# acproject/wsi-segmentation-pipeline

Measured on AMD Instinct MI355X. Metric: patches/sec (256×256×3) whole-slide inference, 1/2/4/8 MI355X + CPU ref, higher is better.
Workload: dtype fp16 + MX-fp6 cross terms (fp32 accumulate); 1 GPU; cfg3: ONE 40000x40000 synthetic slide, tile 256 stride 256 -> 24648 tiles sharded over 1 rank(s) (each holds only its own slide regions: 4.80 GB on rank 0), ResNet-18 trunk + Classifier, fused read+normalise+conv HIP path, 1 all-gather, float64 stitch + softmax; tiles_total=24648, batch=6200, mode=mx, parallelism=tile-shard x1 + 1 all-gather, batches_in_flight=2

## Files before the change

wsi_segmentation_pipeline_amd/csrc/conv.hip:

```cpp
#include "conv_dev.h"
#include "internal.h"

template <int MT, int WM, int WN, int PLANES, bool POST = false>
__global__ __launch_bounds__(WM* WN * 64) void conv_gather_kernel(ConvArgs a) {
    extern __shared__ __attribute__((aligned(16))) char smem[];
    constexpr int BM = WM * MT * 32;
    constexpr int NTHREADS = WM * WN * 64;
    constexpr int PPT = BM * 8 / NTHREADS;
    constexpr int PIX_STEP = NTHREADS / 8;
    const int tid = threadIdx.x, lane = tid & 63, wave = tid >> 6;
    const int wm = wave / WN, wn = wave % WN;
    const int l31 = lane & 31, h = lane >> 5;
    const int nblocks = a.go.C / (WN * 32);
    const int nb = blockIdx.x % nblocks;
    const int mtile = blockIdx.x / nblocks;
    const int q0 = a.go.G + mtile * BM;
    const int ntile = nb * WN + wn;
    const int NC = a.gi.C / PFmt<PLANES>::CPL;
    const int KS = a.ksize, NT = KS * KS, pad = KS / 2;
    const size_t in_pixstride = (size_t)a.gi.C * PFmt<PLANES>::BPC;
    const bf16x8* wbase = (const bf16x8*)a.wpk + (size_t)ntile * NC * NT * 4 * 64 + lane;

    int inq[PPT];
    const int sp = tid & 7;
// ... 22 lines not shown
    for (int c = 0; c < NC; ++c) {
        for (int t = 0; t < NT; ++t) {
            const int toff = (t / KS) * a.gi.P + (t % KS);
            __syncthreads();
#pragma unroll
            for (int k = 0; k < PPT; ++k) {
                const int m = (tid >> 3) + k * PIX_STEP;
                const int s = sp ^ ((m >> 1) & 7);
                const int src = inq[k] < 0 ? 0 : inq[k] + toff;
                *(uint4*)(smem + (size_t)(m * 8 + sp) * 16) =
                    *(const uint4*)((const char*)a.in + (size_t)src * in_pixstride + c * 128 + s * 16);
            }
            bf16x8 wf[4];
#pragma unroll
            for (int f = 0; f < 4; ++f) wf[f] = wbase[((size_t)(c * NT + t) * 4 + f) * 64];
            __syncthreads();
            mfma_line<MT, PLANES>(acc, wf, smem, xbase);
        }
    }
    conv_epilogue<MT, PLANES, POST>(a, acc, q0 + wm * MT * 32, ntile, lane);
}

#ifdef WSI_STUDY
__device__ unsigned long long g_wide_stamps[8];
#define WSTAMP(...) __VA_ARGS__
extern "C" int wsi_study_wide_stamps(unsigned long long* out8, int reset) {
    if (out8 && hipMemcpyFromSymbol(out8, HIP_SYMBOL(g_wide_stamps), sizeof(g_wide_stamps)) != hipSuccess) return WSI_EFAULT;
    if (reset) {
        unsigned long long z[8] = {0};
        if (hipMemcpyToSymbol(HIP_SYMBOL(g_wide_stamps), z, sizeof(z)) != hipSuccess) return WSI_EFAULT;
    }
    return WSI_OK;
}
static __device__ __forceinline__ void wide_stamps_report(int lane, unsigned long long st_begin, unsigned long long st_setup, unsigned long long st_pro,
                                                          unsigned long long st_line, unsigned long long st_tap, unsigned long long st_loop_end) {
    asm volatile("s_waitcnt vmcnt(0)" ::: "memory");
    if (lane == 0 && (blockIdx.x & 63) == 0) {
        const unsigned long long st_end = __builtin_readcyclecounter();
        atomicAdd(&g_wide_stamps[0], 1ull);
        atomicAdd(&g_wide_stamps[1], st_end - st_begin);
        atomicAdd(&g_wide_stamps[2], st_setup - st_begin);
        atomicAdd(&g_wide_stamps[3], st_pro);
        atomicAdd(&g_wide_stamps[4], st_line);
        atomicAdd(&g_wide_stamps[5], st_tap);
        atomicAdd(&g_wide_stamps[6], st_end - st_loop_end);
    }
}
#else
#define WSTAMP(...)
#endif


template <int MT, int WM, int WN, int PLANES, int MINW, bool DENSE, int ABL = 0, bool PAIR = false>
__global__ __launch_bounds__(WM* WN * 64, MINW) void conv3x3s1_slab3_kernel(ConvArgs a) {
    extern __shared__ __attribute__((aligned(16))) char smem[];
    constexpr int BM = WM * MT * 32;
    constexpr int NTHREADS = WM * WN * 64;
    constexpr int RESID_NBUF = MT < 2 ? MT : 2;
    constexpr bool SCHED = MINW < 3;
    const int tid = threadIdx.x, lane = tid & 63;
    if (CONV_STUDY(a, CONV_ABL_DISPATCH_ONLY)) return;
    WSTAMP(const unsigned long long st_begin = __builtin_readcyclecounter(); unsigned long long st_pro = 0, st_line = 0, st_tap = 0, st_a = 0;)
    const int wave = __builtin_amdgcn_readfirstlane(tid >> 6);
    const int wm = wave / WN, wn = wave % WN;
    const int l31 = lane & 31, h = lane >> 5;
    const int nblocks = a.go.C / (WN * 32);
    int nb, mtile;
    if (!conv_tile_of_block(a.flags, nblocks, DENSE ? (a.gi.N * a.gi.H * a.gi.W + BM - 1) / BM : (a.gi.NS + BM - 1) / BM, nb, mtile)) return;
// ... 101 lines not shown
                const int k = t * MT + mt;
                if constexpr (!(ABL & 32)) {
                    if (mt + 1 < MT) xload_m(xf[(k + 1) & 1], xoff[mt + 1] + toff, mt + 1);
                    else if (t < 8) xload_m(xf[(k + 1) & 1], xoff[0] + toff_next, 0);
                }
                if constexpr (SCHED) __builtin_amdgcn_sched_barrier(0);
                const bf16x8(&w)[4] = wbuf[t % 3];
                const bf16x8(&x)[4] = xf[k & 1];
                if constexpr (ABL & 8) {
#pragma unroll
                    for (int f = 0; f < 4; ++f) acc[0][mt][f] += (float)w[f][0] * (float)x[f][0];
                } else if constexpr (PLANES == 3) {
                    acc[0][mt] = mfma_mx6(acc[0][mt], w, x);
                } else if constexpr (PLANES == 2) {
                    mfma_step<2>(acc[0][mt], w, x);
                } else {
#pragma unroll
                    for (int f = 0; f < 4; ++f) acc[0][mt] = mfma_bf16(w[f], x[f], acc[0][mt]);
                }
                if constexpr (SCHED) __builtin_amdgcn_sched_barrier(0);
            }
        }
    }
    WSTAMP(const unsigned long long st_loop_end = __builtin_readcyclecounter();)
    if constexpr (PLANES == 3) {
        if (a.resid) __syncthreads();
        conv_tail_mx<1, MT, RESID_NBUF>(a, acc, qs, valid, ntile, lane, smem + wave * (RESID_NBUF * 4096), slab0);
    } else {
        char* scratch = nullptr;
        if (PLANES == 2 && a.resid && !(a.flags & CONV_RESID_DIRECT)) {
            __syncthreads();
            scratch = smem + wave * 8192;
        }
        conv_epilogue_q<MT, PLANES>(a, acc[0], qs, valid, ntile, lane, scratch);
    }
    WSTAMP(wide_stamps_report(lane, st_begin, st_setup, st_pro, st_line, st_tap, st_loop_end);)
}

long long dense_max_slab_pixels(const ConvArgs& a, int BM) {
    const long long R = (long long)a.gi.N * a.gi.H * a.gi.W;
    const int mtiles = (int)((R + BM - 1) / BM);
    const int HW = a.gi.H * a.gi.W;
    auto pos = [&](long long i) { const long long n = i / HW, rem = i - n * HW; return (long long)a.gi.G + n * a.gi.S + (rem / a.gi.W) * a.gi.P + rem % a.gi.W; };
    auto span = [&](int m) { const long long i0 = (long long)m * BM, i1 = (i0 + BM < R ? i0 + BM : R) - 1; return pos(i1) + a.gi.P + 1 - (pos(i0) - a.gi.P - 1) + 1; };
    long long maxpix = span(mtiles - 1);
    int g = BM, r = HW;
    while (r) { const int t = g % r; g = r; r = t; }
    const int period = HW / g + 1;
    const int scan = mtiles < period ? mtiles : period;
    for (int m = 0; m < scan; ++m) { const long long px = span(m); if (px > maxpix) maxpix = px; }
    return maxpix;
}

size_t conv_slab_lds(long long maxpix, int nthreads, int waves) {
    const size_t lds = (size_t)((maxpix * 8 + nthreads - 1) / nthreads * nthreads) * 16;
    return lds < (size_t)waves * 8192 ? (size_t)waves * 8192 : lds;
}
int conv_grid(int mtiles, int nblocks, int flags) {
    return (flags & CONV_XCD_ORDER) ? (mtiles + 7) / 8 * 8 * nblocks : (flags & CONV_XCD_RANGES) ? (mtiles * nblocks + 7) / 8 * 8 : mtiles * nblocks;
// ... 10 lines not shown
        mtiles = (int)((R + BM - 1) / BM);
        maxpix = (int)dense_max_slab_pixels(a, BM);
    } else {
        mtiles = (a.gi.NS + BM - 1) / BM;
        maxpix = BM + 2 * a.gi.P + 2;
    }
    const size_t lds = conv_slab_lds(maxpix, NTHREADS, WM * WN);
    if (lds > 160 * 1024) return WSI_EINVAL;
    if (PAIR && (!DENSE || MT % 2 || a.gi.W % 64 || ((long long)a.gi.N * a.gi.H * a.gi.W) % BM)) return WSI_EINVAL;
    if (a.in_up) {
        constexpr int CPL = PFmt<PLANES>::CPL;
        if (a.up_c <= 0 || a.up_c % CPL || a.up_c > a.gi.C || (a.up_c < a.gi.C && !a.in) || a.gup.H * 2 != a.gi.H || a.gup.W * 2 != a.gi.W ||
            a.gup.N != a.gi.N || (a.flags & (CONV_IN96 | CONV_RESID96)) || a.in2 ||
            (size_t)pf_alloc_pixels(a.gup.N, a.gup.H, a.gup.W) * a.up_c * PFmt<PLANES>::BPC > (size_t)0x7fffffff)
            return WSI_EINVAL;
    }
    return conv_launch(conv3x3s1_slab3_kernel<MT, WM, WN, PLANES, MINW, DENSE, ABL, PAIR>, conv_grid(mtiles, nblocks, a.flags), NTHREADS, lds, st, a);
}


template <int MINW, int NCT = 0, bool IN96 = true>
__global__ __launch_bounds__(256, MINW) void conv3x3s1_rows_kernel(ConvArgs a) {
    extern __shared__ __attribute__((aligned(16))) char smem[];
    constexpr int MT = 4, WN = 2, BM = 256, NTHREADS = 256, RESID_NBUF = 2;
    const int tid = threadIdx.x, lane = tid & 63;
    WSTAMP(const unsigned long long st_begin = __builtin_readcyclecounter(); unsigned long long st_pro = 0, st_line = 0, st_tap = 0, st_a = 0;)
    const int wave = __builtin_amdgcn_readfirstlane(tid >> 6);
    const int wm = wave / WN, wn = wave % WN;
    const int l31 = lane & 31, h = lane >> 5;
    const int nblocks = a.go.C / (WN * 32);
    int nb, mtile;
    if (!conv_tile_of_block(a.flags & CONV_XCD_RANGES, nblocks, (a.gi.N * a.gi.H * a.gi.W) / BM, nb, mtile)) return;
    const int P = a.gi.P;
    const int ntile = nb * WN + wn;
    const int NC = NCT ? NCT : a.gi.C / 32;
    constexpr bool in96 = IN96;
    const size_t in_pixstride = in96 ? (size_t)96 : (size_t)a.gi.C * 4;
    const int in_line = in96 ? 0 : 128;
    const int p0 = pf_pos_of_index(a.gi, mtile * BM);
    const int slab0 = p0 - P - 1;
    const int npieces = (5 * P + 66) * 8;
    const int xoff0 = wm * 32 + l31;
    const size_t slab_byte0 = (size_t)slab0 * in_pixstride, in_bytes = (size_t)pf_alloc_pixels(a.gi.N, a.gi.H, a.gi.W) * in_pixstride;
    const __amdgpu_buffer_rsrc_t xrs = slab_rsrc(a.in, slab_byte0, in_bytes);
    bool xact;
    const int xvoff = slab_lane_voff96(wave * 64 + lane, (int)in_pixstride, in96, xact);
    const __amdgpu_buffer_rsrc_t wrs = __builtin_amdgcn_make_buffer_rsrc(
// ... 46 lines not shown
        if (c == 0) acc_init_bias<MT>(acc[0], a.bias, ntile, lane);
        xload(xf[0], xoff0);
#pragma unroll
        for (int dx = 0; dx < 3; ++dx) {
#pragma unroll
            for (int j = 0; j < 6; ++j) {
                const int k = dx * 6 + j;
                if (j < 5) xload(xf[(k + 1) & 1], xoff0 + (j + 1) * Pc + dx);
                else if (dx < 2) xload(xf[(k + 1) & 1], xoff0 + dx + 1);
                __builtin_amdgcn_sched_barrier(0);
#pragma unroll
                for (int mt = 0; mt < MT; ++mt) {
                    const int dy = j - mt;
                    if (dy >= 0 && dy < 3) acc[0][mt] = mfma_mx6(acc[0][mt], wbuf[dy], xf[k & 1]);
                }
                __builtin_amdgcn_sched_barrier(0);
                if (j >= 3 && (dx < 2 || (XLINE && c + 1 < NC))) {
                    wload(wbuf[j - 3], dx < 2 ? sline + ((j - 3) * 3 + dx + 1) * 4096 : sline + (9 + (j - 3) * 3) * 4096);
                    __builtin_amdgcn_sched_barrier(0);
                }
            }
        }
    }
    WSTAMP(const unsigned long long st_loop_end = __builtin_readcyclecounter();)
    int qs[MT];
    bool valid[MT];
#pragma unroll
    for (int mt = 0; mt < MT; ++mt) {
        qs[mt] = p0 + mt * P + wm * 32 + l31;
        valid[mt] = true;
    }
    if (a.resid) __syncthreads();
    conv_tail_mx<1, MT, RESID_NBUF>(a, acc, qs, valid, ntile, lane, smem + wave * (RESID_NBUF * 4096), slab0);
    WSTAMP(wide_stamps_report(lane, st_begin, st_setup, st_pro, st_line, st_tap, st_loop_end);)
}

template <int MINW>
static int launch_rows(const ConvArgs& a, hipStream_t st) {
    const bool nc2 = a.gi.C == 64;
    constexpr int BM = 256, NTHREADS = 256;
    if (a.go.C % 64 || a.gi.C % 32 || a.gi.W != 64 || a.gi.H % 4 || a.in2) return WSI_EINVAL;
    const int nblocks = a.go.C / 64;
    const long long R = (long long)a.gi.N * a.gi.H * a.gi.W;
    const int mtiles = (int)(R / BM);
    const size_t lds = conv_slab_lds(5 * a.gi.P + 66, NTHREADS, 4);
    const bool i96 = a.flags & CONV_IN96;
    auto k = nc2 ? (i96 ? conv3x3s1_rows_kernel<MINW, 2, true> : conv3x3s1_rows_kernel<MINW, 2, false>)
                 : (i96 ? conv3x3s1_rows_kernel<MINW, 0, true> : conv3x3s1_rows_kernel<MINW, 0, false>);
    return conv_launch(k, conv_grid(mtiles, nblocks, a.flags & CONV_XCD_RANGES), NTHREADS, lds, st, a);
}


constexpr int L1P_SLAB_PIX = 392;
constexpr int L1P_SLAB = L1P_SLAB_PIX * 128;
constexpr int L1P_STAGE = 16 * 3072;
constexpr int L1P_LDS = 2 * L1P_SLAB + L1P_STAGE;
template <int NCT>
// ... 329 lines not shown
#pragma unroll
            for (int mt = 0; mt < MT; ++mt) {
                const int k = t * MT + mt;
                if constexpr (!(ABL & 32)) {
                    if (mt + 1 < MT) xload(xf[(k + 1) & 1], xoff[mt + 1] + toff, t % 3);
                    else if (t < 8) xload(xf[(k + 1) & 1], xoff[0] + toff_next, (t + 1) % 3);
                }
                __builtin_amdgcn_sched_barrier(0);
                const bf16x8(&x)[4] = xf[k & 1];
#pragma unroll
                for (int nt = 0; nt < NT; ++nt) {
                    mfma_step<PLANES>(acc[nt][mt], wf[nt], x);
                }
            }
            if (t < 8) {
                WSTAMP(st_a = __builtin_readcyclecounter();)
                asm volatile("s_waitcnt vmcnt(0)" ::: "memory");
                __syncthreads();
                WSTAMP(st_tap += __builtin_readcyclecounter() - st_a;)
            }
            kpar ^= 1;
        }
    }
    WSTAMP(const unsigned long long st_loop_end = __builtin_readcyclecounter();)
    int qs[MT];
#pragma unroll
    for (int mt = 0; mt < MT; ++mt) {
        if constexpr (D8) {
            const int i = mtile * BM + wm * MT * 32 + mt * 32 + lpix;
            qs[mt] = pf_pos_of_index(a.gi, valid[mt] ? i : min(mtile * BM + BM, Rtot) - 1);
        } else {
            qs[mt] = xoff[mt] + slab0 + (P + 1);
        }
    }
    if constexpr (PLANES == 3) {
        if (a.in2) {
            const int NC2 = a.in2_c / 32;
            const size_t ps2 = (size_t)a.in2_c * 4;
            const __amdgpu_buffer_rsrc_t xrs2 = slab_rsrc(a.in2, (size_t)slab0 * ps2, (size_t)pf_alloc_pixels(a.gi.N, a.gi.H, a.gi.W) * ps2);
            const int xvoff2 = lane_voff((int)ps2);
            const char* wsrc2 = (const char*)a.wpk2 + (size_t)(nb * NTILES) * NC2 * 4096 + (size_t)(tid & 255) * 16;
#pragma unroll
            for (int nt = 0; nt < NT; ++nt) {
                f32x16 b2[1];
                acc_init_bias<1>(b2, a.bias2, nb * NTILES + wn * NT + nt, lane);
#pragma unroll
                for (int mt = 0; mt < MT; ++mt)
// ... 3 lines not shown
            for (int c = 0; c < NC2; ++c) {
                __syncthreads();
                slab_dma_rounds<NTHREADS, false>(xrs2, xl, wave, npieces, xvoff2, c * 128, RPIX * (int)ps2);
#pragma unroll
                for (int p0 = 0; p0 < NTILES * 256; p0 += NTHREADS) {
                    const int pw = p0 + wave * 64;
                    dma16(wsrc2 + (size_t)((pw >> 8) * NC2 + c) * 4096, wl + pw * 16);
                }
                asm volatile("s_waitcnt vmcnt(0)" ::: "memory");
                __syncthreads();
                bf16x8 wf2[NT][4];
#pragma unroll
                for (int nt = 0; nt < NT; ++nt) wread(wf2[nt], wl, nt);
#pragma unroll
                for (int mt = 0; mt < MT; ++mt) {
                    bf16x8 x2[4];
                    xload(x2, xoff[mt] + (D8 ? 8 : P) + 1);
#pragma unroll
                    for (int nt = 0; nt < NT; ++nt) mfma_step<PLANES>(acc[nt][mt], wf2[nt], x2);
                }
            }
        }
        if (a.resid) __syncthreads();
        conv_tail_mx<NT, MT, RESID_NBUF>(a, acc, qs, valid, nb * NTILES + wn * NT, lane, smem + wave * (RESID_NBUF * 4096), slab0);
    } else {
        char* scratch = nullptr;
        if (PLANES == 2 && a.resid && !(a.flags & CONV_RESID_DIRECT)) {
            __syncthreads();
            scratch = xl + wave * 8192;
        }
#pragma unroll
        for (int nt = 0; nt < NT; ++nt) conv_epilogue_q<MT, PLANES>(a, acc[nt], qs, valid, nb * NTILES + wn * NT + nt, lane, scratch);
    }
    WSTAMP(wide_stamps_report(lane, st_begin, st_setup, st_pro, st_line, st_tap, st_loop_end);)
}


template <int PLANES, int MINW, int ABL = 0, int WM = 2, int WN = 2, int NT = 2, bool D8 = false>
static int launch_wide(const ConvArgs& a, hipStream_t st) {
    constexpr int BM = WM * 128, NTHREADS = WM * WN * 64, BN = WN * NT * 32;
    if (a.go.C % BN) return WSI_EINVAL;
    if constexpr (!D8 && ABL == 0 && WM == 2 && WN == 2 && NT == 2) {
        if (g_routes.wide_d8 && a.gi.W == 8 && a.gi.H == 8) return launch_wide<PLANES, MINW, 0, 2, 2, 2, true>(a, st);
    }
    const int nblocks = a.go.C / BN;
    const long long R = (long long)a.gi.N * a.gi.H * a.gi.W;
    const int mtiles = (int)((R + BM - 1) / BM);
    const size_t xbytes = D8 ? (size_t)(304 + 16) * 128
                             : conv_slab_lds(dense_max_slab_pixels(a, BM), NTHREADS, WM * WN);
    size_t lds = 2 * (BN / 32) * 4096 + xbytes;
    if (PLANES == 3 && lds < (size_t)WM * WN * 4 * 4096) lds = (size_t)WM * WN * 4 * 4096;
    if (lds > 160 * 1024) return WSI_EINVAL;
    return conv_launch(conv3x3s1_wide_kernel<PLANES, MINW, ABL, WM, WN, NT, D8>, conv_grid(mtiles, nblocks, a.flags & CONV_XCD_RANGES), NTHREADS, lds, st, a);
}


template <int MT, int WM, int WN, int PLANES, int MINW, bool FUSE, int PMAX = 34, int ABL = 0>
// ... 471 lines not shown
```

wsi_segmentation_pipeline_amd/csrc/conv_dev.h:

```cpp
#pragma once
#include "common.h"

static __device__ __forceinline__ void dma16(const void* gsrc, char* lds_wave_base) {
    __builtin_amdgcn_global_load_lds((const __attribute__((address_space(1))) void*)gsrc,
                                     (__attribute__((address_space(3))) void*)lds_wave_base, 16, 0, 0);
}

static __device__ __forceinline__ void dma16_buf(__amdgpu_buffer_rsrc_t rs, char* lds_wave_base, int voff, int soff) {
    __builtin_amdgcn_raw_ptr_buffer_load_lds(rs, (__attribute__((address_space(3))) void*)lds_wave_base, 16, voff, soff, 0, 0);
}

static __device__ __forceinline__ unsigned lds_addr_of(const char* p) {
    return (unsigned)(size_t)(const __attribute__((address_space(3))) char*)p;
}
static __device__ __forceinline__ void dma16_asm(const void* gsrc, unsigned lds) {
    unsigned keep;
    asm volatile("s_mov_b32 %0, m0\n\ts_mov_b32 m0, %1\n\ts_nop 0\n\tglobal_load_lds_dwordx4 %2, off\n\ts_mov_b32 m0, %0"
                 : "=&s"(keep) : "s"(lds), "v"(gsrc) : "memory");
}
static __device__ __forceinline__ void dma16_buf_asm(__amdgpu_buffer_rsrc_t rs, unsigned lds, int voff, int soff) {
    unsigned keep;
    asm volatile("s_mov_b32 %0, m0\n\ts_mov_b32 m0, %1\n\ts_nop 0\n\tbuffer_load_dwordx4 %2, %3, %4 offen lds\n\ts_mov_b32 m0, %0"
                 : "=&s"(keep) : "s"(lds), "v"(voff), "s"(rs), "s"(soff) : "memory");
}

static __device__ __forceinline__ void resid_tile_dma(const void* resid, int q_own, size_t pixstride, size_t line_off, int lane, char* dst) {
#pragma unroll
    for (int j = 0; j < 4; ++j) {
        const int pp = 8 * j + (lane >> 3);
        const int q = __shfl(q_own, pp);
        const int sl = (lane & 7) ^ ((pp >> 1) & 7);
        dma16((const char*)resid + (size_t)q * pixstride + line_off + sl * 16, dst + j * 1024);
    }
}

static __device__ __forceinline__ void resid_tile_dma_buf(__amdgpu_buffer_rsrc_t rs, int q_rel, int pixstride, int line_off, int lane, char* dst) {
#pragma unroll
    for (int j = 0; j < 4; ++j) {
        const int pp = 8 * j + (lane >> 3);
        const int q = __shfl(q_rel, pp);
        const int sl = (lane & 7) ^ ((pp >> 1) & 7);
        dma16_buf(rs, dst + j * 1024, q * pixstride + sl * 16, line_off);
    }
}

static __device__ __forceinline__ bool mx96_stored(int s) { return s != 5 && s != 7; }
static __device__ __forceinline__ int mx96_piece(int s) { return s == 6 ? 5 : s; }

static __device__ __forceinline__ void mx96_rebuild_hi6(char* slab, int npix, int tid, int nthreads) {
    for (int Pl = tid; Pl < npix; Pl += nthreads) {
        const int key = (Pl >> 1) & 7;
        char* line = slab + Pl * 128;
        unsigned D[16];
#pragma unroll
        for (int s4 = 0; s4 < 4; ++s4) {
            const u32x4 d = *(const u32x4*)(line + ((s4 ^ key) << 4));
            D[4 * s4] = d[0]; D[4 * s4 + 1] = d[1]; D[4 * s4 + 2] = d[2]; D[4 * s4 + 3] = d[3];
        }
        const int sh = (int)(*(const unsigned*)(line + ((6 ^ key) << 4) + 12) & 255u);
        u32x16 e;
#pragma unroll
        for (int k = 0; k < 16; ++k)
            e[k] = __builtin_amdgcn_perm(D[8 + (k >> 1)], D[k >> 1], (k & 1) ? 0x07060302u : 0x05040100u);
        u32x6 q;
        const float scale = sh ? mx_scale_value(sh) : 1.f;
        asm volatile("v_cvt_scalef32_pk32_fp6_f16 %0, %1, %2" : "=&v"(q) : "v"(e), "v"(scale));
        *(u32x4*)(line + ((5 ^ key) << 4)) = u32x4{q[0], q[1], q[2], q[3]};
        *(u32x4*)(line + ((7 ^ key) << 4)) = u32x4{q[4], q[5], (unsigned)sh, 0u};
    }
}

static __device__ __forceinline__ void resid_tile_dma_buf96(__amdgpu_buffer_rsrc_t rs, int q_rel, int pixstride, int line_off, int lane, char* dst) {
#pragma unroll
    for (int j = 0; j < 4; ++j) {
        const int pp = 8 * j + (lane >> 3);
        const int q = __shfl(q_rel, pp);
        const int sl = (lane & 7) ^ ((pp >> 1) & 7);
        if (mx96_stored(sl)) dma16_buf(rs, dst + j * 1024, q * pixstride + mx96_piece(sl) * 16, line_off);
    }
}

template <int MT, int PLANES, bool POST = false>
static __device__ __forceinline__ void conv_epilogue_q(const ConvArgs& a, f32x16 (&acc)[MT], const int (&qs)[MT],
                                                       const bool (&valid)[MT], int ntile, int lane, char* scratch = nullptr) {
    typedef typename PairElem<PLANES>::T E;
    typedef __attribute__((ext_vector_type(4))) E Ex4;
    const int h = lane >> 5, l31 = lane & 31;
    const size_t pixstride = (size_t)a.go.C * PFmt<PLANES>::BPC;
    const size_t chan_off = (size_t)ntile * (32 * PFmt<PLANES>::BPC) + (size_t)(4 * h) * 2;
    size_t poff[MT], ooff[MT];
#pragma unroll
    for (int mt = 0; mt < MT; ++mt) {
        poff[mt] = (size_t)(valid[mt] ? qs[mt] : a.go.G) * pixstride + chan_off;
        ooff[mt] = a.out_split_pixels ? pf_out_offset(a.go, a.out_split_pixels, valid[mt] ? qs[mt] : a.go.G, pixstride) + chan_off : poff[mt];
    }

    const bool via_lds = PLANES == 2 && a.resid && scratch;
    Ex4 rh[MT][4], rl[MT][4];
    if (via_lds) {
        resid_tile_dma(a.resid, valid[0] ? qs[0] : a.go.G, pixstride, (size_t)ntile * 128, lane, scratch);
    } else if (a.resid) {
// ... 100 lines not shown
    d = __builtin_amdgcn_mfma_f32_32x32x16_f16(__builtin_bit_cast(f16x8, w[1]), __builtin_bit_cast(f16x8, x[1]), d, 0, 0, 0);
    const i32x4 wq = __builtin_bit_cast(i32x4, w[2]), wr = __builtin_bit_cast(i32x4, w[3]);
    const i32x4 xq = __builtin_bit_cast(i32x4, x[2]), xr = __builtin_bit_cast(i32x4, x[3]);
    const i32x8 wa = {wq[0], wq[1], wq[2], wq[3], wr[0], wr[1], wr[2], wr[3]}, xa = {xq[0], xq[1], xq[2], xq[3], xr[0], xr[1], xr[2], xr[3]};
    return __builtin_amdgcn_mfma_scale_f32_32x32x64_f8f6f4(wa, xa, d, 2, 2, 0, wr[2], 0, xr[2]);
}

template <int MT>
static __device__ __forceinline__ void acc_init_bias(f32x16 (&acc)[MT], const float* bias, int ntile, int lane) {
    const int h = lane >> 5;
    float b[16];
#pragma unroll
    for (int g = 0; g < 4; ++g) {
        const f32x4 v = *(const f32x4*)(bias + ntile * 32 + 8 * g + 4 * h);
#pragma unroll
        for (int i = 0; i < 4; ++i) b[4 * g + i] = v[i];
    }
#pragma unroll
    for (int mt = 0; mt < MT; ++mt)
#pragma unroll
        for (int r = 0; r < 16; ++r) acc[mt][r] = b[r];
}

template <int MT, int MTN = MT>
static __device__ __forceinline__ void conv_epilogue_mx(const ConvArgs& a, f32x16 (&acc)[MT], const int (&qs)[MT],
                                                        const bool (&valid)[MT], int ntile, int lane, int mt0 = 0) {
    const int h = lane >> 5;
    const bool o96 = a.flags & CONV_OUT96;
    const size_t pixstride = o96 ? (size_t)96 : (size_t)a.go.C * 4;
    const float lo_clamp = a.relu ? 0.f : -65504.f;
#pragma unroll
    for (int mt = mt0; mt < mt0 + MTN; ++mt) {
        const size_t loff = (size_t)(valid[mt] ? qs[mt] : a.go.G) * pixstride + (o96 ? (size_t)ntile * (size_t)a.plane96 : (size_t)ntile * 128);
        f32x16 v = acc[mt];
        f32x16 hi, lo;
        f16x8 hv[2];
        float mv = 0.f, ml = 0.f;
#pragma unroll
        for (int r = 0; r < 16; r += 2) {
            const float v0 = __builtin_amdgcn_fmed3f(v[r], lo_clamp, 65504.f);
            const float v1 = __builtin_amdgcn_fmed3f(v[r + 1], lo_clamp, 65504.f);
            const f16x2 hh = __builtin_convertvector(f32x2{v0, v1}, f16x2);
            hv[r >> 3][r & 7] = hh[0];
            hv[r >> 3][(r & 7) + 1] = hh[1];
            hi[r] = (float)hh[0];
            hi[r + 1] = (float)hh[1];
            lo[r] = v0 - hi[r];
            lo[r + 1] = v1 - hi[r + 1];
            mv = fmaxf(mv, fmaxf(fabsf(hi[r]), fabsf(hi[r + 1])));
            ml = fmaxf(ml, fmaxf(fabsf(lo[r]), fabsf(lo[r + 1])));
        }
        pair_max2(mv, ml);
        const int sh = mx6_scale_byte(mv), sl = mx6_scale_byte(ml);
        const int sb = h ? sh : sl;
        swap32_halves(lo, hi);
        const u32x6 q = mx6_pack32(lo, hi, sb ? mx_scale_value(sb) : 1.f);
        if (valid[mt] && !CONV_STUDY(a, CONV_ABL_NO_STORE)) {
            char* ol = (char*)a.out + (a.out_split_pixels ? pf_out_offset(a.go, a.out_split_pixels, qs[mt], pixstride) + (size_t)ntile * 128 : loff);
            *(f16x8*)(ol + 32 * h) = hv[0];
            *(f16x8*)(ol + 32 * h + 16) = hv[1];
            if (!o96) {
                *(u32x4*)(ol + MX6_PLANE_LO(0) + 16 * h) = u32x4{q[0], q[1], q[2], q[3]};
                *(u32x4*)(ol + MX6_PLANE_HI(0) + 16 * h) = u32x4{q[4], q[5], (unsigned)sb, 0u};
            } else if (h == 0) {
                *(u32x4*)(ol + 64) = u32x4{q[0], q[1], q[2], q[3]};
                *(u32x4*)(ol + 80) = u32x4{q[4], q[5], (unsigned)sl, (unsigned)sh};
            }
        }
    }
}

template <int NT, int MT, int NBUF>
static __device__ __forceinline__ void conv_tail_mx(const ConvArgs& a, f32x16 (&acc)[NT][MT], const int (&qs)[MT], const bool (&valid)[MT],
                                                    int ntile0, int lane, char* scratch, int slab0) {
    constexpr int T = NT * MT;
    static_assert(MT % NBUF == 0 || NBUF % MT == 0, "a batch is part of one channel tile or whole channel tiles");
    static_assert(NBUF <= T && T % NBUF == 0, "whole batches");
    if (!a.resid) {
#pragma unroll
        for (int nt = 0; nt < NT; ++nt) conv_epilogue_mx<MT>(a, acc[nt], qs, valid, ntile0 + nt, lane);
        return;
    }
    const int h = lane >> 5, l31 = lane & 31;
    const bool r96 = a.flags & CONV_RESID96;
    const int pixstride = r96 ? 96 : a.go.C * 4;
    const size_t rbase = (size_t)slab0 * pixstride, rbytes = (size_t)pf_alloc_pixels(a.go.N, a.go.H, a.go.W) * pixstride;
    const __amdgpu_buffer_rsrc_t rrs = __builtin_amdgcn_make_buffer_rsrc((void*)((const char*)a.resid + rbase), 0,
                                                                          (int)min(rbytes - rbase, (size_t)0x7fffffff), 0x00020000);
    bf16x8 iw[4];
    {
        const int p = mx_line_pos(l31), f0 = mx6_field_of_pos(p);
        f16x8 k0, k1;
#pragma unroll
        for (int j = 0; j < 8; ++j) {
            k0[j] = (p == 8 * h + j) ? (_Float16)1.0f : (_Float16)0.0f;
            k1[j] = (p == 16 + 8 * h + j) ? (_Float16)1.0f : (_Float16)0.0f;
        }
        unsigned q[6];
#pragma unroll
        for (int d = 0; d < 6; ++d) {
            const int bit = 6 * f0 + 3 - 32 * d;
            q[d] = (h == 0 && bit >= 0 && bit < 32) ? (1u << (bit & 31)) : 0u;
        }
        iw[0] = __builtin_bit_cast(bf16x8, k0);
        iw[1] = __builtin_bit_cast(bf16x8, k1);
        iw[2] = __builtin_bit_cast(bf16x8, u32x4{q[0], q[1], q[2], q[3]});
        iw[3] = __builtin_bit_cast(bf16x8, u32x4{q[4], q[5], 127u, 0u});
    }
    auto rdma = [&](int k) {
        const int nt = k / MT, mt = k % MT;
        int qr = qs[mt] - slab0;
        asm volatile("" : "+v"(qr));
        if (r96) {
            const __amdgpu_buffer_rsrc_t prs = __builtin_amdgcn_make_buffer_rsrc(
                (void*)((const char*)a.resid + (size_t)(ntile0 + nt) * (size_t)a.plane96 + rbase), 0, (int)min(rbytes - rbase, (size_t)0x7fffffff), 0x00020000);
            resid_tile_dma_buf96(prs, qr, pixstride, 0, lane, scratch + (k % NBUF) * 4096);
        }
        else resid_tile_dma_buf(rrs, qr, pixstride, (ntile0 + nt) * 128, lane, scratch + (k % NBUF) * 4096);
    };
    const int xb = l31 * 128 + ((h ^ ((l31 >> 1) & 7)) << 4);
#pragma unroll
    for (int k = 0; k < NBUF; ++k) rdma(k);
#pragma unroll
    for (int b0 = 0; b0 < T; b0 += NBUF) {
        asm volatile("s_waitcnt vmcnt(0)" ::: "memory");
#pragma unroll
        for (int k = b0; k < b0 + NBUF; ++k) {
            const char* t = scratch + (k % NBUF) * 4096;
            bf16x8 x[4];
#pragma unroll
            for (int f = 0; f < 4; ++f) x[f] = *(const bf16x8*)(t + (xb ^ (f << 5)));
            if (r96 && h) {
                x[2] = __builtin_bit_cast(bf16x8, u32x4{0u, 0u, 0u, 0u});
                x[3] = x[2];
            }
            acc[k / MT][k % MT] = mfma_mx6(acc[k / MT][k % MT], iw, x);
        }
        if (b0 + NBUF < T) {
            asm volatile("s_waitcnt lgkmcnt(0)" ::: "memory");
#pragma unroll
            for (int k = b0 + NBUF; k < b0 + 2 * NBUF; ++k) rdma(k);
        }
        if constexpr (NBUF >= MT) {
#pragma unroll
            for (int nt = b0 / MT; nt < (b0 + NBUF) / MT; ++nt) conv_epilogue_mx<MT>(a, acc[nt], qs, valid, ntile0 + nt, lane);
        } else {
            conv_epilogue_mx<MT, NBUF>(a, acc[b0 / MT], qs, valid, ntile0 + b0 / MT, lane, b0 % MT);
        }
    }
}

template <int MT, int PLANES, bool POST = false>
static __device__ __forceinline__ void conv_epilogue(const ConvArgs& a, f32x16 (&acc)[MT], int q_base, int ntile,
                                                     int lane) {
    int qs[MT];
    bool valid[MT];
#pragma unroll
    for (int mt = 0; mt < MT; ++mt) {
        qs[mt] = q_base + mt * 32 + (lane & 31);
        valid[mt] = pf_is_pixel(a.go, qs[mt]);
    }
    conv_epilogue_q<MT, PLANES, POST>(a, acc, qs, valid, ntile, lane);
}

template <int MT, int PLANES>
static __device__ __forceinline__ void conv_epilogue_any(const ConvArgs& a, f32x16 (&acc)[MT], int q_base, int ntile, int lane) {
    if constexpr (PLANES == 3) {
        int qs[MT];
        bool valid[MT];
#pragma unroll
// ... 144 lines not shown
```

wsi_segmentation_pipeline_amd/csrc/conv_pp.hip:

```cpp
#include "conv_dev.h"
#include "internal.h"

#define PP_BARRIER() do { asm volatile("s_waitcnt lgkmcnt(0)\n\ts_barrier" ::: "memory"); __builtin_amdgcn_sched_barrier(0); } while (0)
#define PP_BARRIER_VM() do { asm volatile("s_waitcnt vmcnt(0) lgkmcnt(0)\n\ts_barrier" ::: "memory"); __builtin_amdgcn_sched_barrier(0); } while (0)

#ifdef WSI_STUDY
#define PP_STAMP(x) do { if constexpr (STAMP) { unsigned long long t_; asm volatile("s_memtime %0\n\ts_waitcnt lgkmcnt(0)" : "=s"(t_) :: "memory"); x; } } while (0)
#else
#define PP_STAMP(x) do { } while (0)
#endif

template <int PLANES, int WM, int WN, int MT, bool STAMP = false, int DMODE = 0, bool PRIO = false>
__global__ __launch_bounds__(512, 2) void conv3x3s1_pp_kernel(ConvArgs a, int xbytes) {
    extern __shared__ __attribute__((aligned(16))) char smem[];
    constexpr int NT = 2, BM = WM * MT * 32, NTILES = WN * NT, WB = NTILES * 4096;
    constexpr int NF = 4;
    constexpr int RESID_NBUF = 4;
    static_assert(WM * WN == 8, "eight waves: two groups of four, one wave of each group per SIMD");
    char* const wl = smem;
    char* const xl = smem + 2 * WB;
    const int tid = threadIdx.x, lane = tid & 63;
    const int wave = __builtin_amdgcn_readfirstlane(tid >> 6);
    const int grp = wave >> 2;
    const int wm = wave / WN, wn = wave % WN;
// ... 114 lines not shown
            for (int mt = 0; mt < MT; ++mt)
#pragma unroll
                for (int nt = 0; nt < NT; ++nt) mfma_step<PLANES>(acc[nt][mt], wf[nt], xf[mt]);
#pragma unroll
            for (int mt = 0; mt < MT; ++mt) asm volatile("" : "+v"(acc[0][mt]), "+v"(acc[1][mt]));
            if constexpr (PRIO) __builtin_amdgcn_s_setprio(0);
            PP_STAMP(tsum[2] += t_ - tprev; tprev = t_);
            if (grp == 0 && DMODE != 1) asm volatile("s_waitcnt vmcnt(0)" ::: "memory");
            PP_BARRIER();
            PP_STAMP(tsum[3] += t_ - tprev; tprev = t_);
        }
    }
#ifdef WSI_STUDY
    if constexpr (STAMP) {
        if ((blockIdx.x == 0 || blockIdx.x == 300) && lane == 0 && a.out2) {
            unsigned long long* o = (unsigned long long*)a.out2 + ((blockIdx.x ? 1 : 0) * 8 + wave) * 6;
            for (int k = 0; k < 6; ++k) o[k] = tsum[k];
        }
    }
#endif
    if (grp == 0) PP_BARRIER();
    if constexpr (PLANES == 3) {
        constexpr int NBUF = RESID_NBUF % MT ? MT : (RESID_NBUF < NT * MT ? RESID_NBUF : NT * MT);
        conv_tail_mx<NT, MT, NBUF>(a, acc, qs, valid, nb * NTILES + wn * NT, lane, smem + wave * (RESID_NBUF * 4096), slab0);
    } else {
        char* scratch = nullptr;
        if (PLANES == 2 && a.resid && !(a.flags & CONV_RESID_DIRECT)) scratch = xl + wave * 8192;
#pragma unroll
        for (int nt = 0; nt < NT; ++nt) conv_epilogue_q<MT, PLANES>(a, acc[nt], qs, valid, nb * NTILES + wn * NT + nt, lane, scratch);
    }
}

template <int PLANES, int WM, int WN, int MT, bool STAMP = false, int DMODE = 0, bool PRIO = false>
static int launch_pp(const ConvArgs& a, hipStream_t st) {
    constexpr int BM = WM * MT * 32, BN = WN * 2 * 32;
    if (a.go.C % BN) return WSI_EINVAL;
    const int nblocks = a.go.C / BN;
    const long long R = (long long)a.gi.N * a.gi.H * a.gi.W;
    const int mtiles = (int)((R + BM - 1) / BM);
    const size_t xbytes = conv_slab_lds(dense_max_slab_pixels(a, BM), 64, 4);
    size_t lds = 2 * (size_t)(BN / 32) * 4096 + 2 * xbytes;
    if (PLANES == 3 && lds < 8 * 4 * 4096) lds = 8 * 4 * 4096;
    if (lds > 160 * 1024 || xbytes > 65536) return WSI_EINVAL;
    auto k = conv3x3s1_pp_kernel<PLANES, WM, WN, MT, STAMP, DMODE, PRIO>;
    static bool lds_ok = false;
    if (!lds_ok) {
        if (hipFuncSetAttribute((const void*)k, hipFuncAttributeMaxDynamicSharedMemorySize, 160 * 1024) != hipSuccess) return WSI_EINVAL;
// ... 28 lines not shown
```

Baseline: 123,400 patches/s.

## Compact residual tile staging to 96 bytes per pixel and pipeline tail MFMA reads

The MX residual tail now stages each residual tile into LDS as six 16-byte pieces per pixel (96 B) in three DMA rounds, instead of four rounds of swizzled 128 B lines. This merges the plain and 96-byte DMA helpers and shrinks the per-tile LDS scratch. The tail also rebuilds the identity weights per batch rather than keeping them live, double-buffers the LDS reads ahead of each MFMA with scheduling barriers, and runs the epilogue per tile with opaque lane/offset values to limit register pressure. The aim is less global and LDS traffic and a shorter epilogue critical path. The cost is more instructions for the per-batch weight setup and a riskier, hand-scheduled tail. Study-only timing stamps for the tail are also added.

```diff
diff --git a/wsi_segmentation_pipeline_amd/csrc/conv.hip b/wsi_segmentation_pipeline_amd/csrc/conv.hip
--- a/wsi_segmentation_pipeline_amd/csrc/conv.hip
+++ b/wsi_segmentation_pipeline_amd/csrc/conv.hip
@@ -68,18 +68,19 @@
 }
 
 #ifdef WSI_STUDY
-__device__ unsigned long long g_wide_stamps[8];
+__device__ unsigned long long g_wide_stamps[16];
 #define WSTAMP(...) __VA_ARGS__
-extern "C" int wsi_study_wide_stamps(unsigned long long* out8, int reset) {
-    if (out8 && hipMemcpyFromSymbol(out8, HIP_SYMBOL(g_wide_stamps), sizeof(g_wide_stamps)) != hipSuccess) return WSI_EFAULT;
+extern "C" int wsi_study_wide_stamps(unsigned long long* out16, int reset) {
+    if (out16 && hipMemcpyFromSymbol(out16, HIP_SYMBOL(g_wide_stamps), sizeof(g_wide_stamps)) != hipSuccess) return WSI_EFAULT;
     if (reset) {
-        unsigned long long z[8] = {0};
+        unsigned long long z[16] = {0};
         if (hipMemcpyToSymbol(HIP_SYMBOL(g_wide_stamps), z, sizeof(z)) != hipSuccess) return WSI_EFAULT;
     }
     return WSI_OK;
 }
 static __device__ __forceinline__ void wide_stamps_report(int lane, unsigned long long st_begin, unsigned long long st_setup, unsigned long long st_pro,
-                                                          unsigned long long st_line, unsigned long long st_tap, unsigned long long st_loop_end) {
+                                                          unsigned long long st_line, unsigned long long st_tap, unsigned long long st_loop_end,
+                                                          const TailStamps& ts) {
     asm volatile("s_waitcnt vmcnt(0)" ::: "memory");
     if (lane == 0 && (blockIdx.x & 63) == 0) {
         const unsigned long long st_end = __builtin_readcyclecounter();
@@ -90,6 +91,12 @@
         atomicAdd(&g_wide_stamps[4], st_line);
         atomicAdd(&g_wide_stamps[5], st_tap);
         atomicAdd(&g_wide_stamps[6], st_end - st_loop_end);
+        atomicAdd(&g_wide_stamps[8], ts.first);
+        atomicAdd(&g_wide_stamps[9], ts.wait);
+        atomicAdd(&g_wide_stamps[10], ts.mfma);
+        atomicAdd(&g_wide_stamps[11], ts.req);
+        atomicAdd(&g_wide_stamps[12], ts.enc);
+        atomicAdd(&g_wide_stamps[13], ts.store);
     }
 }
 #else
@@ -237,10 +244,10 @@
             }
         }
     }
-    WSTAMP(const unsigned long long st_loop_end = __builtin_readcyclecounter();)
+    WSTAMP(const unsigned long long st_loop_end = __builtin_readcyclecounter(); TailStamps tail_st = {};)
     if constexpr (PLANES == 3) {
         if (a.resid) __syncthreads();
-        conv_tail_mx<1, MT, RESID_NBUF>(a, acc, qs, valid, ntile, lane, smem + wave * (RESID_NBUF * 4096), slab0);
+        conv_tail_mx<1, MT, RESID_NBUF>(a, acc, qs, valid, ntile, lane, smem + wave * (RESID_NBUF * RESID_TILE_LDS), slab0 WSTAMP(, &tail_st));
     } else {
         char* scratch = nullptr;
         if (PLANES == 2 && a.resid && !(a.flags & CONV_RESID_DIRECT)) {
@@ -249,7 +256,7 @@
         }
         conv_epilogue_q<MT, PLANES>(a, acc[0], qs, valid, ntile, lane, scratch);
     }
-    WSTAMP(wide_stamps_report(lane, st_begin, st_setup, st_pro, st_line, st_tap, st_loop_end);)
+    WSTAMP(wide_stamps_report(lane, st_begin, st_setup, st_pro, st_line, st_tap, st_loop_end, tail_st);)
 }
 
 long long dense_max_slab_pixels(const ConvArgs& a, int BM) {
@@ -306,7 +313,8 @@
 template <int MINW, int NCT = 0, bool IN96 = true>
 __global__ __launch_bounds__(256, MINW) void conv3x3s1_rows_kernel(ConvArgs a) {
     extern __shared__ __attribute__((aligned(16))) char smem[];
-    constexpr int MT = 4, WN = 2, BM = 256, NTHREADS = 256, RESID_NBUF = 2;
+    constexpr int MT = 4, WN = 2, BM = 256, NTHREADS = 256;
+    constexpr int RESID_NBUF = 2;
     const int tid = threadIdx.x, lane = tid & 63;
     WSTAMP(const unsigned long long st_begin = __builtin_readcyclecounter(); unsigned long long st_pro = 0, st_line = 0, st_tap = 0, st_a = 0;)
     const int wave = __builtin_amdgcn_readfirstlane(tid >> 6);
@@ -399,7 +407,7 @@
             }
         }
     }
-    WSTAMP(const unsigned long long st_loop_end = __builtin_readcyclecounter();)
+    WSTAMP(const unsigned long long st_loop_end = __builtin_readcyclecounter(); TailStamps tail_st = {};)
     int qs[MT];
     bool valid[MT];
 #pragma unroll
@@ -408,8 +416,8 @@
         valid[mt] = true;
     }
     if (a.resid) __syncthreads();
-    conv_tail_mx<1, MT, RESID_NBUF>(a, acc, qs, valid, ntile, lane, smem + wave * (RESID_NBUF * 4096), slab0);
-    WSTAMP(wide_stamps_report(lane, st_begin, st_setup, st_pro, st_line, st_tap, st_loop_end);)
+    conv_tail_mx<1, MT, RESID_NBUF, true>(a, acc, qs, valid, ntile, lane, smem + wave * (RESID_NBUF * RESID_TILE_LDS), slab0 WSTAMP(, &tail_st));
+    WSTAMP(wide_stamps_report(lane, st_begin, st_setup, st_pro, st_line, st_tap, st_loop_end, tail_st);)
 }
 
 template <int MINW>
@@ -785,7 +793,7 @@
             kpar ^= 1;
         }
     }
-    WSTAMP(const unsigned long long st_loop_end = __builtin_readcyclecounter();)
+    WSTAMP(const unsigned long long st_loop_end = __builtin_readcyclecounter(); TailStamps tail_st = {};)
     int qs[MT];
 #pragma unroll
     for (int mt = 0; mt < MT; ++mt) {
@@ -835,7 +843,7 @@
             }
         }
         if (a.resid) __syncthreads();
-        conv_tail_mx<NT, MT, RESID_NBUF>(a, acc, qs, valid, nb * NTILES + wn * NT, lane, smem + wave * (RESID_NBUF * 4096), slab0);
+        conv_tail_mx<NT, MT, RESID_NBUF>(a, acc, qs, valid, nb * NTILES + wn * NT, lane, smem + wave * (RESID_NBUF * RESID_TILE_LDS), slab0 WSTAMP(, &tail_st));
     } else {
         char* scratch = nullptr;
         if (PLANES == 2 && a.resid && !(a.flags & CONV_RESID_DIRECT)) {
@@ -845,7 +853,7 @@
 #pragma unroll
         for (int nt = 0; nt < NT; ++nt) conv_epilogue_q<MT, PLANES>(a, acc[nt], qs, valid, nb * NTILES + wn * NT + nt, lane, scratch);
     }
-    WSTAMP(wide_stamps_report(lane, st_begin, st_setup, st_pro, st_line, st_tap, st_loop_end);)
+    WSTAMP(wide_stamps_report(lane, st_begin, st_setup, st_pro, st_line, st_tap, st_loop_end, tail_st);)
 }
 
 
diff --git a/wsi_segmentation_pipeline_amd/csrc/conv_dev.h b/wsi_segmentation_pipeline_amd/csrc/conv_dev.h
--- a/wsi_segmentation_pipeline_amd/csrc/conv_dev.h
+++ b/wsi_segmentation_pipeline_amd/csrc/conv_dev.h
@@ -31,16 +31,6 @@
         const int q = __shfl(q_own, pp);
         const int sl = (lane & 7) ^ ((pp >> 1) & 7);
         dma16((const char*)resid + (size_t)q * pixstride + line_off + sl * 16, dst + j * 1024);
-    }
-}
-
-static __device__ __forceinline__ void resid_tile_dma_buf(__amdgpu_buffer_rsrc_t rs, int q_rel, int pixstride, int line_off, int lane, char* dst) {
-#pragma unroll
-    for (int j = 0; j < 4; ++j) {
-        const int pp = 8 * j + (lane >> 3);
-        const int q = __shfl(q_rel, pp);
-        const int sl = (lane & 7) ^ ((pp >> 1) & 7);
-        dma16_buf(rs, dst + j * 1024, q * pixstride + sl * 16, line_off);
     }
 }
 
@@ -70,13 +60,13 @@
     }
 }
 
-static __device__ __forceinline__ void resid_tile_dma_buf96(__amdgpu_buffer_rsrc_t rs, int q_rel, int pixstride, int line_off, int lane, char* dst) {
-#pragma unroll
-    for (int j = 0; j < 4; ++j) {
-        const int pp = 8 * j + (lane >> 3);
+constexpr int RESID_TILE_LDS = 32 * 96;
+static __device__ __forceinline__ void resid_tile_dma_buf(__amdgpu_buffer_rsrc_t rs, int q_rel, int pixstride, int line_off, int lane, bool l96, char* dst) {
+#pragma unroll
+    for (int r = 0; r < 3; ++r) {
+        const int g = 64 * r + lane, pp = g / 6, c = g - 6 * pp;
         const int q = __shfl(q_rel, pp);
-        const int sl = (lane & 7) ^ ((pp >> 1) & 7);
-        if (mx96_stored(sl)) dma16_buf(rs, dst + j * 1024, q * pixstride + mx96_piece(sl) * 16, line_off);
+        dma16_buf(rs, dst + r * 1024, q * pixstride + (c == 5 && !l96 ? 6 : c) * 16, line_off);
     }
 }
 
@@ -223,16 +213,31 @@
         for (int r = 0; r < 16; ++r) acc[mt][r] = b[r];
 }
 
-template <int MT, int MTN = MT>
+#ifdef WSI_STUDY
+#define TSTAMP(...) __VA_ARGS__
+struct TailStamps { unsigned long long t, first, wait, mfma, req, enc, store; };
+static __device__ __forceinline__ void tstamp(TailStamps* ts, unsigned long long TailStamps::*slot) {
+    if (!ts) return;
+    const unsigned long long now = __builtin_readcyclecounter();
+    if (slot) ts->*slot += now - ts->t;
+    ts->t = now;
+}
+#else
+#define TSTAMP(...)
+#endif
+
+template <int MT, int MTN = MT, bool PER_TILE = false>
 static __device__ __forceinline__ void conv_epilogue_mx(const ConvArgs& a, f32x16 (&acc)[MT], const int (&qs)[MT],
-                                                        const bool (&valid)[MT], int ntile, int lane, int mt0 = 0) {
+                                                        const bool (&valid)[MT], int ntile, int lane, int mt0 = 0 TSTAMP(, TailStamps* ts = nullptr)) {
     const int h = lane >> 5;
     const bool o96 = a.flags & CONV_OUT96;
     const size_t pixstride = o96 ? (size_t)96 : (size_t)a.go.C * 4;
     const float lo_clamp = a.relu ? 0.f : -65504.f;
 #pragma unroll
     for (int mt = mt0; mt < mt0 + MTN; ++mt) {
-        const size_t loff = (size_t)(valid[mt] ? qs[mt] : a.go.G) * pixstride + (o96 ? (size_t)ntile * (size_t)a.plane96 : (size_t)ntile * 128);
+        int qo = valid[mt] ? qs[mt] : a.go.G;
+        if constexpr (PER_TILE) asm volatile("" : "+v"(qo));
+        const size_t loff = (size_t)qo * pixstride + (o96 ? (size_t)ntile * (size_t)a.plane96 : (size_t)ntile * 128);
         f32x16 v = acc[mt];
         f32x16 hi, lo;
         f16x8 hv[2];
@@ -256,97 +261,124 @@
         const int sb = h ? sh : sl;
         swap32_halves(lo, hi);
         const u32x6 q = mx6_pack32(lo, hi, sb ? mx_scale_value(sb) : 1.f);
+        TSTAMP(tstamp(ts, &TailStamps::enc);)
         if (valid[mt] && !CONV_STUDY(a, CONV_ABL_NO_STORE)) {
-            char* ol = (char*)a.out + (a.out_split_pixels ? pf_out_offset(a.go, a.out_split_pixels, qs[mt], pixstride) + (size_t)ntile * 128 : loff);
-            *(f16x8*)(ol + 32 * h) = hv[0];
-            *(f16x8*)(ol + 32 * h + 16) = hv[1];
+            int ln = lane;
+            if constexpr (PER_TILE) asm volatile("" : "+v"(ln));
+            const int hb = (ln >> 5) * 16;
+            char* ol = (char*)a.out + (a.out_split_pixels ? pf_out_offset(a.go, a.out_split_pixels, qo, pixstride) + (size_t)ntile * 128 : loff) + hb;
+            *(f16x8*)(ol + hb) = hv[0];
+            *(f16x8*)(ol + hb + 16) = hv[1];
             if (!o96) {
-                *(u32x4*)(ol + MX6_PLANE_LO(0) + 16 * h) = u32x4{q[0], q[1], q[2], q[3]};
-                *(u32x4*)(ol + MX6_PLANE_HI(0) + 16 * h) = u32x4{q[4], q[5], (unsigned)sb, 0u};
+                *(u32x4*)(ol + MX6_PLANE_LO(0)) = u32x4{q[0], q[1], q[2], q[3]};
+                *(u32x4*)(ol + MX6_PLANE_HI(0)) = u32x4{q[4], q[5], (unsigned)sb, 0u};
             } else if (h == 0) {
                 *(u32x4*)(ol + 64) = u32x4{q[0], q[1], q[2], q[3]};
                 *(u32x4*)(ol + 80) = u32x4{q[4], q[5], (unsigned)sl, (unsigned)sh};
             }
         }
-    }
-}
-
-template <int NT, int MT, int NBUF>
+        TSTAMP(tstamp(ts, &TailStamps::store);)
+    }
+}
+
+template <int NT, int MT, int NBUF, bool PER_TILE_PLAIN = false>
 static __device__ __forceinline__ void conv_tail_mx(const ConvArgs& a, f32x16 (&acc)[NT][MT], const int (&qs)[MT], const bool (&valid)[MT],
-                                                    int ntile0, int lane, char* scratch, int slab0) {
+                                                    int ntile0, int lane, char* scratch, int slab0 TSTAMP(, TailStamps* ts = nullptr)) {
     constexpr int T = NT * MT;
     static_assert(MT % NBUF == 0 || NBUF % MT == 0, "a batch is part of one channel tile or whole channel tiles");
     static_assert(NBUF <= T && T % NBUF == 0, "whole batches");
+    TSTAMP(tstamp(ts, nullptr);)
     if (!a.resid) {
 #pragma unroll
-        for (int nt = 0; nt < NT; ++nt) conv_epilogue_mx<MT>(a, acc[nt], qs, valid, ntile0 + nt, lane);
+        for (int nt = 0; nt < NT; ++nt) conv_epilogue_mx<MT, MT, PER_TILE_PLAIN>(a, acc[nt], qs, valid, ntile0 + nt, lane, 0 TSTAMP(, ts));
         return;
     }
-    const int h = lane >> 5, l31 = lane & 31;
     const bool r96 = a.flags & CONV_RESID96;
     const int pixstride = r96 ? 96 : a.go.C * 4;
     const size_t rbase = (size_t)slab0 * pixstride, rbytes = (size_t)pf_alloc_pixels(a.go.N, a.go.H, a.go.W) * pixstride;
-    const __amdgpu_buffer_rsrc_t rrs = __builtin_amdgcn_make_buffer_rsrc((void*)((const char*)a.resid + rbase), 0,
-                                                                          (int)min(rbytes - rbase, (size_t)0x7fffffff), 0x00020000);
-    bf16x8 iw[4];
-    {
-        const int p = mx_line_pos(l31), f0 = mx6_field_of_pos(p);
-        f16x8 k0, k1;
-#pragma unroll
-        for (int j = 0; j < 8; ++j) {
-            k0[j] = (p == 8 * h + j) ? (_Float16)1.0f : (_Float16)0.0f;
-            k1[j] = (p == 16 + 8 * h + j) ? (_Float16)1.0f : (_Float16)0.0f;
-        }
-        unsigned q[6];
-#pragma unroll
-        for (int d = 0; d < 6; ++d) {
-            const int bit = 6 * f0 + 3 - 32 * d;
-            q[d] = (h == 0 && bit >= 0 && bit < 32) ? (1u << (bit & 31)) : 0u;
-        }
-        iw[0] = __builtin_bit_cast(bf16x8, k0);
-        iw[1] = __builtin_bit_cast(bf16x8, k1);
-        iw[2] = __builtin_bit_cast(bf16x8, u32x4{q[0], q[1], q[2], q[3]});
-        iw[3] = __builtin_bit_cast(bf16x8, u32x4{q[4], q[5], 127u, 0u});
-    }
     auto rdma = [&](int k) {
         const int nt = k / MT, mt = k % MT;
-        int qr = qs[mt] - slab0;
-        asm volatile("" : "+v"(qr));
-        if (r96) {
-            const __amdgpu_buffer_rsrc_t prs = __builtin_amdgcn_make_buffer_rsrc(
-                (void*)((const char*)a.resid + (size_t)(ntile0 + nt) * (size_t)a.plane96 + rbase), 0, (int)min(rbytes - rbase, (size_t)0x7fffffff), 0x00020000);
-            resid_tile_dma_buf96(prs, qr, pixstride, 0, lane, scratch + (k % NBUF) * 4096);
-        }
-        else resid_tile_dma_buf(rrs, qr, pixstride, (ntile0 + nt) * 128, lane, scratch + (k % NBUF) * 4096);
+        int qr = qs[mt] - slab0, ln = lane;
+        asm volatile("" : "+v"(qr), "+v"(ln));
+        const __amdgpu_buffer_rsrc_t rs = __builtin_amdgcn_make_buffer_rsrc(
+            (void*)((const char*)a.resid + (r96 ? (size_t)(ntile0 + nt) * (size_t)a.plane96 : (size_t)0) + rbase), 0,
+            (int)min(rbytes - rbase, (size_t)0x7fffffff), 0x00020000);
+        resid_tile_dma_buf(rs, qr, pixstride, r96 ? 0 : (ntile0 + nt) * 128, ln, r96, scratch + (k % NBUF) * RESID_TILE_LDS);
     };
-    const int xb = l31 * 128 + ((h ^ ((l31 >> 1) & 7)) << 4);
+    auto xread = [&](bf16x8(&x)[4], int k) {
+        int ln = lane;
+        asm volatile("" : "+v"(ln));
+        const char* t = scratch + (k % NBUF) * RESID_TILE_LDS + (ln & 31) * 96;
+        x[0] = *(const bf16x8*)(t + (ln >> 5) * 16);
+        x[1] = *(const bf16x8*)(t + (ln >> 5) * 16 + 32);
+        x[2] = *(const bf16x8*)(t + 64);
+        x[3] = *(const bf16x8*)(t + 80);
+    };
+    auto xzero = [&](bf16x8(&x)[4]) {
+        int ln = lane;
+        asm volatile("" : "+v"(ln));
+        u32x4 v2 = __builtin_bit_cast(u32x4, x[2]), v3 = __builtin_bit_cast(u32x4, x[3]);
+#pragma unroll
+        for (int d = 0; d < 4; ++d) {
+            v2[d] = ln < 32 ? v2[d] : 0u;
+            v3[d] = ln < 32 ? v3[d] : 0u;
+        }
+        x[2] = __builtin_bit_cast(bf16x8, v2);
+        x[3] = __builtin_bit_cast(bf16x8, v3);
+    };
 #pragma unroll
     for (int k = 0; k < NBUF; ++k) rdma(k);
 #pragma unroll
     for (int b0 = 0; b0 < T; b0 += NBUF) {
+        bf16x8 iw[4];
+        {
+            int ln = lane;
+            asm volatile("" : "+v"(ln));
+            const int h = ln >> 5, p = mx_line_pos(ln & 31), f0 = mx6_field_of_pos(p);
+            f16x8 k0, k1;
+#pragma unroll
+            for (int j = 0; j < 8; ++j) {
+                k0[j] = (p == 8 * h + j) ? (_Float16)1.0f : (_Float16)0.0f;
+                k1[j] = (p == 16 + 8 * h + j) ? (_Float16)1.0f : (_Float16)0.0f;
+            }
+            unsigned q[6];
+#pragma unroll
+            for (int d = 0; d < 6; ++d) {
+                const int bit = 6 * f0 + 3 - 32 * d;
+                q[d] = (h == 0 && bit >= 0 && bit < 32) ? (1u << (bit & 31)) : 0u;
+            }
+            iw[0] = __builtin_bit_cast(bf16x8, k0);
+            iw[1] = __builtin_bit_cast(bf16x8, k1);
+            iw[2] = __builtin_bit_cast(bf16x8, u32x4{q[0], q[1], q[2], q[3]});
+            iw[3] = __builtin_bit_cast(bf16x8, u32x4{q[4], q[5], 127u, 0u});
+        }
         asm volatile("s_waitcnt vmcnt(0)" ::: "memory");
+        TSTAMP(tstamp(ts, b0 ? &TailStamps::wait : &TailStamps::first);)
+        bf16x8 x[2][4];
+        xread(x[0], b0);
 #pragma unroll
         for (int k = b0; k < b0 + NBUF; ++k) {
-            const char* t = scratch + (k % NBUF) * 4096;
-            bf16x8 x[4];
-#pragma unroll
-            for (int f = 0; f < 4; ++f) x[f] = *(const bf16x8*)(t + (xb ^ (f << 5)));
-            if (r96 && h) {
-                x[2] = __builtin_bit_cast(bf16x8, u32x4{0u, 0u, 0u, 0u});
-                x[3] = x[2];
-            }
-            acc[k / MT][k % MT] = mfma_mx6(acc[k / MT][k % MT], iw, x);
-        }
+            if (k + 1 < b0 + NBUF) xread(x[(k + 1 - b0) & 1], k + 1);
+            __builtin_amdgcn_sched_barrier(0);
+            xzero(x[(k - b0) & 1]);
+            acc[k / MT][k % MT] = mfma_mx6(acc[k / MT][k % MT], iw, x[(k - b0) & 1]);
+            __builtin_amdgcn_sched_barrier(0);
+        }
+        TSTAMP(tstamp(ts, &TailStamps::mfma);)
         if (b0 + NBUF < T) {
             asm volatile("s_waitcnt lgkmcnt(0)" ::: "memory");
 #pragma unroll
             for (int k = b0 + NBUF; k < b0 + 2 * NBUF; ++k) rdma(k);
+            TSTAMP(tstamp(ts, &TailStamps::req);)
         }
         if constexpr (NBUF >= MT) {
 #pragma unroll
-            for (int nt = b0 / MT; nt < (b0 + NBUF) / MT; ++nt) conv_epilogue_mx<MT>(a, acc[nt], qs, valid, ntile0 + nt, lane);
+            for (int k = b0; k < b0 + NBUF; ++k) {
+                conv_epilogue_mx<MT, 1, true>(a, acc[k / MT], qs, valid, ntile0 + k / MT, lane, k % MT TSTAMP(, ts));
+                __builtin_amdgcn_sched_barrier(0);
+            }
         } else {
-            conv_epilogue_mx<MT, NBUF>(a, acc[b0 / MT], qs, valid, ntile0 + b0 / MT, lane, b0 % MT);
+            conv_epilogue_mx<MT, NBUF, true>(a, acc[b0 / MT], qs, valid, ntile0 + b0 / MT, lane, b0 % MT TSTAMP(, ts));
         }
     }
 }
diff --git a/wsi_segmentation_pipeline_amd/csrc/conv_pp.hip b/wsi_segmentation_pipeline_amd/csrc/conv_pp.hip
--- a/wsi_segmentation_pipeline_amd/csrc/conv_pp.hip
+++ b/wsi_segmentation_pipeline_amd/csrc/conv_pp.hip
@@ -160,7 +160,7 @@
     if (grp == 0) PP_BARRIER();
     if constexpr (PLANES == 3) {
         constexpr int NBUF = RESID_NBUF % MT ? MT : (RESID_NBUF < NT * MT ? RESID_NBUF : NT * MT);
-        conv_tail_mx<NT, MT, NBUF>(a, acc, qs, valid, nb * NTILES + wn * NT, lane, smem + wave * (RESID_NBUF * 4096), slab0);
+        conv_tail_mx<NT, MT, NBUF>(a, acc, qs, valid, nb * NTILES + wn * NT, lane, smem + wave * (RESID_NBUF * RESID_TILE_LDS), slab0);
     } else {
         char* scratch = nullptr;
         if (PLANES == 2 && a.resid && !(a.flags & CONV_RESID_DIRECT)) scratch = xl + wave * 8192;
```

New measurement: 124,500 patches/s, median of 6. About the same (+0.9%).
